# atlas-jj/ORB-SLAM-free-space-carving

Hardware: AMD Instinct MI355X
Metric: Mpix*KF/s fused (640x480xN_KF) (higher is better)
Workload: dtype f32

## Files before the change

### orb-slam-free-space-carving_amd/csrc/sdm_device.h

```cpp
#pragma once
#include <hip/hip_runtime.h>
#include <float.h>
#include <stddef.h>
#include <stdint.h>

#include "sdm_c.h"

namespace sdm {

struct KfMeta {
    float fx, fy, cx, cy;
    float Tcw[12];
    float I_stddev;
    int uploaded;
    int pad[2];
};

struct RefConst {
    int slot;
    float fx, fy, cx, cy;
    float mind, maxd;
    int act_count;
};

// ... 271 lines not shown
    return __builtin_fmaf(e, r, r);
}

#ifndef SDM_K1_OPT_ATAN_RCP
#define SDM_K1_OPT_ATAN_RCP 1
#endif
__device__ __forceinline__ float fast_atan2_deg_x1(float y)
{
    const float scale = (float)(180.0 / 3.14159265358979323846);
    const float p1 = 0.9997878412794807f * scale;
    const float p3 = -0.3258083974640975f * scale;
    const float p5 = 0.1555786518463281f * scale;
    const float p7 = -0.04432655554792128f * scale;
    float ay = fabsf(y);
    float a, c, c2;
    if (1.0f >= ay) {
        c = ay;
        c2 = c * c;
        a = (((p7 * c2 + p5) * c2 + p3) * c2 + p1) * c;
    } else {
#if SDM_K1_OPT_ATAN_RCP
        c = rcp_exact(ay + (float)DBL_EPSILON);
#else
        c = 1.0f / (ay + (float)DBL_EPSILON);
#endif
        c2 = c * c;
        a = 90.f - (((p7 * c2 + p5) * c2 + p3) * c2 + p1) * c;
    }
    if (y < 0) a = 360.f - a;
    return a;
}

#ifndef SDM_K1_OPT
#define SDM_K1_OPT 0x17fa27f
#endif

constexpr int PCV_FLOATS = 20;
constexpr int CV_RX = 9, CV_RZ = 12, CV_TX = 15, CV_TZ = 16, CV_ROT = 17, CV_ISTD = 18;
static_assert(offsetof(PairConst, Rx) == 4 * CV_RX && offsetof(PairConst, Rz) == 4 * CV_RZ && offsetof(PairConst, tx) == 4 * CV_TX &&
                  offsetof(PairConst, tz) == 4 * CV_TZ && offsetof(PairConst, rot) == 4 * CV_ROT &&
                  offsetof(PairConst, istd) == 4 * CV_ISTD && offsetof(PairConst, Ry) == 4 * PCV_FLOATS,
              "the CV_* indices follow PairConst");

__device__ __forceinline__ float match_cost1(float pe2, float ge2, const DevParams& prm)
{
    double s = (double)pe2 + (double)ge2 * prm.inv_theta;
    const unsigned lo = (unsigned)__double2loint(s), hi = (unsigned)__double2hiint(s);
    const bool risky = (((lo & 0x1FFFFFFFu) - 0x0FFFFF00u) <= 0x200u) | ((hi - 0x39C00000u) >= (0x46200000u - 0x39C00000u));
    if (__builtin_expect(risky, 0)) s = (double)pe2 + (double)ge2 / prm.theta_var;
    return (float)s;
}

constexpr float INV_THETA_DEFAULT_F = (float)(1.0 / 0.23);
constexpr unsigned COST_BAND = 16u;
__device__ __forceinline__ float match_cost_ref(float pe2, float ge2, const DevParams& prm)
{
    return (float)((double)pe2 + (double)ge2 / prm.theta_var);
}
__device__ __forceinline__ float match_cost_approx(float pe2, float ge2) { return __builtin_fmaf(ge2, INV_THETA_DEFAULT_F, pe2); }

__device__ __forceinline__ float lerp_w0(float yf)
{
#if SDM_K1_OPT & 0x10
    return 1.0f - __builtin_amdgcn_fractf(yf);
#else
    return (floorf(yf) + 1.0f) - yf;
#endif
// ... 179 lines not shown
    in = in && fx > 0.0f && fy > 0.0f && mind > 0.0f && maxd > 0.0f && tx != 0.0f && W >= 2 && H >= 2 && W <= 65536 && H <= 65536;
    if (!in) return 0;
    const Box xp0 = box_out((0.0f - cx) / fx, ((float)(W - 1) - cx) / fx);
    const Box xp1 = box_out((0.0f - cy) / fy, ((float)(H - 1) - cy) / fy);
    const Box rxxp = box_add(box_add(box_mul(box_pt(Rx[0]), xp0), box_mul(box_pt(Rx[1]), xp1)), box_pt(Rx[2]));
    const Box rzxp = box_add(box_add(box_mul(box_pt(Rz[0]), xp0), box_mul(box_pt(Rz[1]), xp1)), box_pt(Rz[2]));
    int bits = 0;
    {
        bool ok = fx * 0x1p-25f * fabsf(tx) * (1.0f - 0x1p-20f) >= QB_NUM_LO;
        const float ds[2] = {mind, maxd};
        for (int k = 0; k < 2; k++) {
            const Box xk = box_add(box_mul(rxxp, box_pt(ds[k])), box_pt(tx));
            const Box zk = box_add(box_mul(rzxp, box_pt(ds[k])), box_pt(tz));
            ok = ok && box_divisor_ok(zk) && box_mag_hi(box_mul(box_pt(fx), xk)) <= QB_NUM_HI;
        }
        if (ok) bits |= 8;
    }
    {
        const float w = (float)W;
        const Box ucx = box_add(Box{-QB_U_SPAN * w, (QB_U_SPAN + 1.0f) * w}, box_pt(-cx));
        const Box num = box_add(box_mul(rzxp, ucx), box_neg(box_mul(box_pt(fx), rxxp)));
        const Box den = box_add(box_mul(box_pt(-tz), ucx), box_mul(box_pt(fx), box_pt(tx)));
        const float nvar = 2 * istd * istd;
        const float lb = fminf(0x1p-50f * fx * fabsf(Rx[2]), rzxp.lo * 0x1p-25f * fabsf(cx)) * (1.0f - 0x1p-20f);
        bool ok = box_divisor_ok(den) && box_mag_hi(num) <= QB_NUM_HI && Rx[2] != 0.0f && cx != 0.0f && rzxp.lo >= 0x1p-10f &&
                  lb >= QB_NUM_LO && quot_input_ok(istd) && istd > 0.0f && nvar >= QB_NUM_LO && nvar <= QB_NUM_HI;
        const float root = (1002.0f + 1.4143f * istd) / (QB_U_SPAN * w) * (1.0f + 0x1p-10f);
        const unsigned eb = max((__float_as_uint(root * root) >> 23) + 1u, 97u);
        ok = ok && eb < (QB_DWIN_END >> 23);
        if (ok) bits |= 16 | (int)(eb << 8);
    }
    return bits;
}

struct ScanState {
    float old_err, best_pe, best_ge;
    int best_pixel;
};

struct ScanConst {
    const char* nbase;
    unsigned W16;
    float hlim_b;
    float ab, cb, pixel, grad1, th_line, ang_pi_rot, gate_lim;
    int hi;
};
template <bool STATS, bool CLEAN>
__device__ __forceinline__ void scan_candidate(const ScanConst& q, int uj, float yf, const float4& r, const DevParams& prm,
                                               ScanState& S, SearchStats* st)
{
    if (r.x < prm.lambdaG) return;
#if SDM_ABLATE == 4
    if (r.z > S.old_err) { S.best_pixel = uj; S.old_err = r.z; }
    return;
#endif
    const float d2 = r.y - q.th_line;
    const float d3 = r.y - q.ang_pi_rot;
    bool fail;
    if (CLEAN) {
#if SDM_K1_OPT & 0x04
        fail = gate2_fails_fast1(d2) | gate3_fails_fast1(d3);
#else
        fail = gate2_fails_fast(d2) | gate3_fails_fast(d3);
#endif
    } else {
        fail = gate2_fails_k(d2, prm.g2c) | gate3_fails_k(d3, prm.g3lo, prm.g3span);
// ... 530 lines not shown
    t_one = 1.0 / s2;
    const bool safe = (s2 > 1.0e-60) & (s2 < 1.0e60) & (ar > 1.0e-30f) & (ar < 1.0e30f);
    t_rho = safe ? div_by_with_rcp((double)rho, s2, t_one) : (double)rho / s2;
#endif
}
__device__ __forceinline__ void fusion_accum(float rho, float sg, float& pjsj, float& rsj)
{
    double t_rho, t_one;
    fusion_terms(rho, sg, t_rho, t_one);
    pjsj = (float)((double)pjsj + t_rho);
    rsj = (float)((double)rsj + t_one);
}
constexpr unsigned FD_SG_LO = 77u << 23, FD_SG_END = 177u << 23;
__device__ __forceinline__ bool fusion_accum_try(float rho, float sg, float& pjsj, float& rsj)
{
    if ((__float_as_uint(sg) - FD_SG_LO) >= (FD_SG_END - FD_SG_LO)) return false;
    const double sd = (double)sg;
    const double y = rcp_newton_f64(sd * sd, __builtin_amdgcn_rcpf(sg * sg));
    float np, nr;
    const bool okp = decided_sum((double)pjsj, (double)rho * y, np);
    const bool okr = decided_sum((double)rsj, y, nr);
    if (!(okp & okr)) return false;
    pjsj = np;
    rsj = nr;
    return true;
}
__device__ __forceinline__ void fusion_accum_decided(float rho, float sg, float& pjsj, float& rsj)
{
#if SDM_K1_OPT & 0x400000
    if (fusion_accum_try(rho, sg, pjsj, rsj)) return;
#endif
    fusion_accum(rho, sg, pjsj, rsj);
}

__device__ __forceinline__ float2 fusion_tail_ref(float pjsj, float rsj) { return make_float2(pjsj / rsj, sqrtf(1 / rsj)); }
__device__ __forceinline__ bool fusion_tail_window(float pjsj, float rsj)
{
    return ((__float_as_uint(pjsj) - QUOT_MAG_LO) <= (QUOT_MAG_HI - QUOT_MAG_LO)) &
           ((__float_as_uint(rsj) - QUOT_MAG_LO) <= (QUOT_MAG_HI - QUOT_MAG_LO));
}
__device__ __forceinline__ float2 fusion_tail_fast(float pjsj, float rsj)
{
    const float r = rcp_fast(rsj);
    const float rs = __builtin_amdgcn_rsqf(r);
    const float y0 = r * rs, hs = 0.5f * rs;
    return make_float2(quot_fast(pjsj, rsj, r), __builtin_fmaf(__builtin_fmaf(-y0, y0, r), hs, y0));
}
__device__ __forceinline__ float2 fusion_tail(float pjsj, float rsj)
{
#if SDM_K1_OPT & 0x800000
    if (fusion_tail_window(pjsj, rsj)) return fusion_tail_fast(pjsj, rsj);
#endif
    return fusion_tail_ref(pjsj, rsj);
}

__device__ __forceinline__ bool gt_1em6(float x) { return x > __uint_as_float(0x358637bdu); }
__device__ __forceinline__ bool lt_1em6(float x) { return x <= __uint_as_float(0x358637bdu); }

__device__ __forceinline__ float safe_rcp_sq(float s)
{
    float s2 = s * s;
    bool ok = (s2 >= 1.0e-30f) && (s2 <= 1.0e30f);
    return ok ? __builtin_amdgcn_rcpf(s2) : __builtin_nanf("");
}

__device__ __forceinline__ bool chi_test_fast(float a, float b, float sa, float sb, float ra, float rb)
// ... 10 lines not shown
{
    float d = ha.x - hb.x;
    float num = d * d;
    float approx = num * ha.y + num * hb.y;
    if (approx < 5.9896f) return true;
    if (approx > 5.9904f) return false;
    return chi_test(ha.x, hb.x, sa, *sb_ptr);
}

__device__ __forceinline__ bool fuse_column(const float2* hyp, int stride, int nh, int lambdaN,
                                            float& rho_o, float& sigma_o)
{
    unsigned long long bestmask = 0;
    int best = 0;
    for (int a = 0; a < nh; a++) {
        float2 ha = hyp[a * stride];
        const float ra = safe_rcp_sq(ha.y);
        unsigned long long m = 0;
        for (int b = 0; b < nh; b++) {
            float2 hb = hyp[b * stride];
            if (chi_test_fast(ha.x, hb.x, ha.y, hb.y, ra, safe_rcp_sq(hb.y))) m |= 1ull << b;
        }
        int cnt = __popcll(m);
        if (cnt > best) {
            best = cnt;
            bestmask = m;
        }
    }
    if (best < lambdaN) return false;
    float pjsj = 0.f, rsj = 0.f;
    for (int b = 0; b < nh; b++) {
        if (!((bestmask >> b) & 1ull)) continue;
        float2 hb = hyp[b * stride];
        fusion_accum_decided(hb.x, hb.y, pjsj, rsj);
    }
    const float2 res = fusion_tail(pjsj, rsj);
    rho_o = res.x;
    sigma_o = res.y;
    return true;
}

}
```

### orb-slam-free-space-carving_amd/csrc/sdm_engine.hip

```cpp
#include <hip/hip_runtime.h>

#include <algorithm>
#include <atomic>
#include <chrono>
#include <cmath>
#include <condition_variable>
#include <cstdio>
#include <cstdlib>
#include <cstring>
#include <limits>
#include <map>
#include <mutex>
#include <string>
#include <thread>
#include <new>
#include <vector>

#include "sdm_c.h"
#include "sdm_kernels.h"
#include "sdm_extract.h"
#include "sdm_support.h"
#include "sdm_priors.h"
#include "sdm_covis.h"
#include "sdm_voxel.h"
// ... 2546 lines not shown
        if (hipMalloc(&d_pc, sizeof(PairConst) * blocks * BLOCK) != hipSuccess) {
            (void)hipFree(d_patch);
            return fail(SDM_EHIP, "selftest scratch allocation failed");
        }
        hipLaunchKernelGGL(k_selftest_k4, dim3(blocks), dim3(BLOCK), 0, c->stream, 2048, d_patch, d_pc, c->d_stats + 5,
                           c->d_stats + 6, which == 9 ? 1 : 0);
        hipError_t e = hipGetLastError();
        if (e == hipSuccess) e = hipMemcpyAsync(out, c->d_stats + 5, sizeof(unsigned long long) * 2, hipMemcpyDeviceToHost, c->stream);
        if (e == hipSuccess) e = hipStreamSynchronize(c->stream);
        (void)hipFree(d_patch);
        (void)hipFree(d_pc);
        if (e != hipSuccess) return fail(SDM_EHIP, hipGetErrorString(e));
        HIP_TRY(hipMemsetAsync(c->d_stats, 0, sizeof(unsigned long long) * STATS_WORDS, c->stream));
        return SDM_OK;
    } else if (which == 6) {
        hipLaunchKernelGGL(k_selftest_rcp, dim3(4096), dim3(BLOCK), 0, c->stream, c->d_stats + 5, c->d_stats + 6);
    } else if (which == 8) {
        hipLaunchKernelGGL(k_selftest_scan_ids, dim3(4096), dim3(BLOCK), 0, c->stream, c->d_stats + 5, c->d_stats + 6);
    } else if (which == 10) {
        hipLaunchKernelGGL(k_selftest_atan_x1, dim3(4096), dim3(BLOCK), 0, c->stream, c->d_stats + 5, c->d_stats + 6);
    } else if (which == 3) {
        hipLaunchKernelGGL(k_selftest_gates, dim3(4096), dim3(BLOCK), 0, c->stream, c->dprm, c->d_stats + 5, c->d_stats + 6);
    } else if (which == 11) {
        hipLaunchKernelGGL(k_selftest_quot_boxes, dim3(4096), dim3(BLOCK), 0, c->stream, 4096, c->d_stats + 5, c->d_stats + 6);
    } else if (which == 13) {
        hipLaunchKernelGGL(k_selftest_ustar, dim3(ST_DEC_BLOCKS), dim3(BLOCK), 0, c->stream, c->dprm.inv_theta, ST13_ITERS,
                           c->d_stats + 5, c->d_stats + 6);
    } else if (which == 14) {
        hipLaunchKernelGGL(k_selftest_fusion_decided, dim3(ST_DEC_BLOCKS), dim3(BLOCK), 0, c->stream, ST14_ITERS, c->d_stats + 5,
                           c->d_stats + 6);
    } else if (which == 15) {
        hipLaunchKernelGGL(k_selftest_fusion_tail, dim3(ST_DEC_BLOCKS), dim3(BLOCK), 0, c->stream, ST15_ITERS, c->d_stats + 5,
                           c->d_stats + 6);
    } else if (which == 12) {
        const sdm_ctx::TableKey& key = c->sets[c->cur_set].key;
        if (!key.valid || !key.has_consts || !c->d_pairs) return fail(SDM_EINVAL, "no pair constants staged");
        const int np = key.n_ref * key.n;
        hipLaunchKernelGGL(k_selftest_pair_bits, dim3((np + BLOCK - 1) / BLOCK), dim3(BLOCK), 0, c->stream, c->d_pairs, np,
                           c->d_stats + 5, c->d_stats + 6);
    } else if (which == 16 || which == 17 || which == 18) {
        const unsigned long long* keys = nullptr;
        unsigned long long cap = 0;
        if (which == 18) {
            if (!c->vox_last_keys) return fail(SDM_ESTATE, "no per-call voxel table: sdm_extract_points_voxel* first");
            keys = c->vox_last_keys, cap = c->vox_last_cap;
        } else {
            if (!c->vmap.open) return fail(SDM_ESTATE, "no open voxel map");
            if (which == 16) keys = c->vmap.tb.keys, cap = c->vmap.cap;
            else if (c->vmap.obs.d_table) keys = c->vmap.obs.tb.keys, cap = c->vmap.obs.cap;
        }
        if (cap)
            launch_sliced(c, (long long)((cap + BLOCK - 1) / BLOCK), [&](long long b0, unsigned g) {
                hipLaunchKernelGGL(k_selftest_table_layout, dim3(g), dim3(BLOCK), 0, c->stream, keys, cap,
                                   (unsigned long long)b0 * BLOCK, c->d_stats + 5);
            });
    } else {
        return fail(SDM_EINVAL, "unknown selftest");
    }
    HIP_TRY(hipGetLastError());
    HIP_TRY(hipMemcpyAsync(out, c->d_stats + 5, sizeof(unsigned long long) * 2, hipMemcpyDeviceToHost, c->stream));
    HIP_TRY(hipStreamSynchronize(c->stream));
    HIP_TRY(hipMemsetAsync(c->d_stats, 0, sizeof(unsigned long long) * STATS_WORDS, c->stream));
    return SDM_OK;
}

int sdm_enable_timing(sdm_ctx* c, int on)
{
    if (!c) return fail(SDM_EINVAL, "null context");
    c->timing_on = on != 0;
    return SDM_OK;
}

// ... 75 lines not shown
```

### orb-slam-free-space-carving_amd/csrc/sdm_kernels.h

```cpp
#pragma once
#include "sdm_device.h"
#include "sdm_ingest.h"

namespace sdm {

#ifndef SDM_INTRA_COMPACT
#define SDM_INTRA_COMPACT 1
#endif

struct TileGeom {
    int W, H, tiles_x, tiles_y, ntiles;
};

__host__ __device__ inline TileGeom make_geom(int W, int H)
{
    TileGeom g;
    g.W = W;
    g.H = H;
    g.tiles_x = (W + TILE_W - 1) / TILE_W;
    g.tiles_y = (H + TILE_H - 1) / TILE_H;
    g.ntiles = g.tiles_x * g.tiles_y;
    return g;
}
__host__ inline int grid_blocks(const TileGeom& g, int n_ref) { return 8 * ((g.ntiles + 7) / 8) * n_ref; }
// ... 109 lines not shown
    if (idx >= n_ref * n) return;
    int r = idx / n, j = idx - r * n;
    KfMeta m1 = meta[ref_slots[r]];
    KfMeta m2 = meta[nbr_slots[idx]];
    PairConst pc;
    float R21[9], t21[3];
    pair_geometry(m1, m2, pc.F, R21, t21);
    for (int i = 0; i < 3; i++) {
        pc.Rx[i] = R21[i];
        pc.Ry[i] = R21[3 + i];
        pc.Rz[i] = R21[6 + i];
    }
    pc.tx = t21[0];
    pc.ty = t21[1];
    pc.tz = t21[2];
    pc.rot = rot ? rot[idx] : 0.0f;
    pc.istd = m2.I_stddev;
    pc.nbr_slot = nbr_slots[idx];
    pc.nfx = m2.fx;
    pc.nfy = m2.fy;
    pc.ncx = m2.cx;
    pc.ncy = m2.cy;
    pc.clean = ((theta_bad[ref_slots[r]] == 0 && theta_bad[nbr_slots[idx]] == 0 && pc.rot >= -360.0f && pc.rot <= 360.0f) ? 1 : 0) |
               (line_quot_safe(pc.F) ? 2 : 0);
    {
        float umin, umax;
        search_range(m1.fx, m1.cx, pc.Rx[2], pc.Rz[2], pc.tx, pc.tz, mind ? mind[r] : 0.f, maxd ? maxd[r] : 0.f, W, umin, umax);
        if (!(umax - umin < (float)MASK_HINT_L)) pc.clean |= 4;
    }
#if SDM_K1_OPT & 0x1c0000
    pc.clean |= quot_boxes(pc.Rx, pc.Rz, pc.tx, pc.tz, pc.istd, m1.fx, m1.fy, m1.cx, m1.cy, mind ? mind[r] : 0.f, maxd ? maxd[r] : 0.f,
                           W, H);
#endif
    {
        const float s = 1.0f + 0x1p-20f;
        const float X0 = fmaxf(fabsf(m1.cx), fabsf((float)(W - 1) - m1.cx)) / fabsf(m1.fx) * s;
        const float X1 = fmaxf(fabsf(m1.cy), fabsf((float)(H - 1) - m1.cy)) / fabsf(m1.fy) * s;
        k4_proj_bounds(pc, X0, X1);
    }
    pairs[idx] = pc;
    if (j == 0) {
        RefConst rc;
        rc.slot = ref_slots[r];
        rc.fx = m1.fx;
        rc.fy = m1.fy;
        rc.cx = m1.cx;
        rc.cy = m1.cy;
        rc.mind = mind ? mind[r] : 0.f;
        rc.maxd = maxd ? maxd[r] : 0.f;
        rc.act_count = act_counts[ref_slots[r]];
        refs[r] = rc;
    }
}

__global__ void k_ref_setup(const KfMeta* __restrict__ meta, const int* __restrict__ ref_slots,
                            const int* __restrict__ act_counts, int n_ref, RefConst* __restrict__ refs)
{
    int r = blockIdx.x * blockDim.x + threadIdx.x;
    if (r >= n_ref) return;
    KfMeta m = meta[ref_slots[r]];
    RefConst rc;
    rc.slot = ref_slots[r];
    rc.fx = m.fx;
    rc.fy = m.fy;
    rc.cx = m.cx;
    rc.cy = m.cy;
// ... 50 lines not shown
        const float sa = sgm[a * K1_PX + p];
        unsigned c = (sa * sa > 0.0f) ? 1u : 0u;
        for (int bb = a + 1; bb < n; bb++) {
            const float2 hb = hyp[bb * K1_PX + p];
            if (chi_test_lazy(ha, hb, sa, &sgm[bb * K1_PX + p])) {
                c++;
                atomicAdd(&cnt[(bb >> 2) * K1_PX + p], 1u << (8 * (bb & 3)));
            }
        }
        atomicAdd(&cnt[(a >> 2) * K1_PX + p], c << (8 * (a & 3)));
    }
}
__device__ __forceinline__ bool k1_fuse_counted(const float2* hyp, const float* sgm, const unsigned* cnt, unsigned long long vm,
                                                int n, int p, int lambdaN, float2& result)
{
    unsigned best = 0;
    int besta = 0;
    for (int a = 0; a < n; a++) {
        if (!((vm >> a) & 1ull)) continue;
        const unsigned c = (cnt[(a >> 2) * K1_PX + p] >> (8 * (a & 3))) & 0xffu;
        if (c > best) {
            best = c;
            besta = a;
        }
    }
    if ((int)best < lambdaN) return false;
    const float2 ha = hyp[besta * K1_PX + p];
    const float sa = sgm[besta * K1_PX + p];
    float pjsj = 0.f, rsj = 0.f;
    for (int bb = 0; bb < n; bb++) {
        if (!((vm >> bb) & 1ull)) continue;
        const float2 hb = hyp[bb * K1_PX + p];
        const bool in = (bb == besta) ? (sa * sa > 0.0f) : chi_test_lazy(ha, hb, sa, &sgm[bb * K1_PX + p]);
        if (in) fusion_accum_decided(hb.x, sgm[bb * K1_PX + p], pjsj, rsj);
    }
    result = fusion_tail(pjsj, rsj);
    return true;
}

#ifndef SDM_K1_EU_MIN
#define SDM_K1_EU_MIN 8
#endif
#ifndef SDM_K1_LB
#define SDM_K1_LB __launch_bounds__(K1_BLOCK) __attribute__((amdgpu_waves_per_eu(SDM_K1_EU_MIN, 8)))
#endif
template <bool STATS, bool MASK>
__global__ SDM_K1_LB void k_search_fuse(const float4* __restrict__ rec, long long plane,
                                                       const RefConst* __restrict__ refs,
                                                       const PairConst* __restrict__ pairs, int n_ref, int n,
                                                       int W, int H, int max_chunks, DevParams prm,
                                                       const unsigned* __restrict__ act, float2* __restrict__ pool,
                                                       unsigned long long* __restrict__ stats, OpenList open_list,
                                                       const unsigned* __restrict__ gmask, int mrow)
{
    extern __shared__ __align__(16) unsigned char smem_raw[];
    float2* hyp = reinterpret_cast<float2*>(smem_raw);
    float* sgm = reinterpret_cast<float*>(hyp + (size_t)n * K1_PX);
    unsigned* cnt = reinterpret_cast<unsigned*>(sgm + (size_t)n * K1_PX);
    const int cnt_words = max((n + 3) >> 2, K1_OUTLIER_ROWS);
    unsigned long long* pmask = reinterpret_cast<unsigned long long*>(cnt + (size_t)cnt_words * K1_PX);
    unsigned long long* set0 = pmask + K1_BLOCK;
    unsigned* cnt0 = reinterpret_cast<unsigned*>(set0 + K1_PX);
    unsigned* xbase = cnt0 + K1_PX;

    const int b = blockIdx.x;
    const int i8 = b >> 3;
    const int cl = i8 / n_ref;
    const int ref = i8 - cl * n_ref;
    const int chunk = cl * 8 + (b & 7);
    if (chunk >= max_chunks) return;
    const RefConst rc = refs[ref];
    if (chunk * K1_PX >= rc.act_count) return;
    const int tid = threadIdx.x, p = tid & (K1_PX - 1);
    const int w = __builtin_amdgcn_readfirstlane(tid >> 6);
    const int t = chunk * K1_PX + p;
    const bool on = t < rc.act_count;
    const float4* __restrict__ rrec = rec + (long long)rc.slot * plane;

    int x = 2, y = 2;
    float pixel = 0.f, grad1 = 0.f, th_pi = 0.f, xp0 = 0.f, xp1 = 0.f;
    if (on) {
        unsigned xy = act[(long long)rc.slot * plane + t];
        x = (int)(xy & 0xffffu);
        y = (int)(xy >> 16);
        float4 r = rrec[y * W + x];
        pixel = (float)(int)(__float_as_uint(r.w) & 0xffu);
        grad1 = r.x;
        th_pi = r.y;
        xp0 = ((float)x - rc.cx) / rc.fx;
        xp1 = ((float)y - rc.cy) / rc.fy;
    }
    SearchStats st = {0, 0, 0};
    MaskStats ms = {0, 0, 0};
    MaskView mv;
    mv.row_pitch = (unsigned)mrow * MASK_WORD_BYTES;
    const PairConst* __restrict__ pcs = pairs + (long long)ref * n;
    const float rcvb[4] = {rc.fx, rc.cx, rc.mind, rc.maxd};
    const float* __restrict__ rcv = rcvb;
    unsigned long long mymask = 0;
    for (int j = w; j < n; j += K1_WAVES) {
        const PairConst* __restrict__ pc = pcs + j;
        const float4* __restrict__ nrec = rec + (long long)pc->nbr_slot * plane;
        float2 h = make_float2(__builtin_inff(), 1.0f);
#if SDM_K1_OPT & 0x1000
        {
            float rho, sigma, bu, bv;
            const float* __restrict__ cv = reinterpret_cast<const float*>(pc);
            bool ok = epipolar_search<STATS, true>(nrec, W, H, cv, rcv, pc->clean, on, x, y, pixel, grad1, th_pi, xp0, xp1, prm,
                                                   rho, sigma, bu, bv, &st);
            if (ok && __float_as_uint(rho) < 0x7f800000u) {
                h = make_float2(rho, sigma);
                mymask |= 1ull << j;
            }
        }
#else
        if (on) {
            float rho, sigma, bu, bv;
            const float* __restrict__ cv = reinterpret_cast<const float*>(pc);
            mv.base = (MASK && gmask) ? reinterpret_cast<const char*>(gmask + (long long)pc->nbr_slot * H * MASK_PLANES * mrow) : nullptr;
            bool ok = epipolar_search<STATS, false, MASK>(nrec, W, H, cv, rcv, pc->clean, true, x, y, pixel, grad1, th_pi, xp0, xp1, prm, rho,
                                             sigma, bu, bv, &st, mv, &ms);
            if (ok && __float_as_uint(rho) < 0x7f800000u) {
                h = make_float2(rho, sigma);
                mymask |= 1ull << j;
            }
        }
#endif
        hyp[j * K1_PX + p] = make_float2(h.x, safe_rcp_sq(h.y));
        sgm[j * K1_PX + p] = h.y;
    }
    for (int q = w; q < cnt_words; q += K1_WAVES) cnt[q * K1_PX + p] = 0u;
    if (w == 0) {
        set0[p] = 0ull;
        cnt0[p] = 0u;
    }
    pmask[tid] = mymask;
    __syncthreads();

    unsigned long long vm = 0;
#pragma unroll
    for (int q = 0; q < K1_WAVES; q++) vm |= pmask[q * K1_PX + p];
#if SDM_ABLATE == 1
    const int nh = 0;
    if (vm == 0x123456789ull) pool[0] = make_float2(1.f, 1.f);
#else
    const int nh = __popcll(vm);
#endif
    const bool go = nh > prm.lambdaN;
    const int a0 = (int)__ffsll((long long)vm) - 1;
    bool self0 = false;
    if (go) {
        const float2 ha = hyp[a0 * K1_PX + p];
        const float sa = sgm[a0 * K1_PX + p];
        self0 = sa * sa > 0.0f;
        unsigned c = 0;
        for (int bb = w; bb < n; bb += K1_WAVES) {
            const float2 hb = hyp[bb * K1_PX + p];
            if (bb != a0 && chi_test_lazy(ha, hb, sa, &sgm[bb * K1_PX + p])) c++;
        }
        if (c) atomicAdd(&cnt0[p], c);
    }
    __syncthreads();
#if SDM_ABLATE == 9
    bool settled = false;
    const bool few = false;
    const unsigned long long S0 = 0ull;
    const int s0 = 0;
#else
    bool settled = go && self0 && (int)cnt0[p] + 1 == nh;
    const bool more = go && !settled && self0;
    unsigned long long S0 = settled ? vm : 0ull;
    if (__builtin_amdgcn_ballot_w64(more) != 0ull) {
        if (more) {
            const float2 ha = hyp[a0 * K1_PX + p];
            const float sa = sgm[a0 * K1_PX + p];
            unsigned long long m = 0;
            for (int bb = w; bb < n; bb += K1_WAVES) {
                const float2 hb = hyp[bb * K1_PX + p];
                if (bb != a0 && chi_test_lazy(ha, hb, sa, &sgm[bb * K1_PX + p])) m |= 1ull << bb;
            }
            if (m) atomicOr(&set0[p], m);
        }
        __syncthreads();
        if (more) S0 = set0[p] | (1ull << a0);
    }
    const int s0 = __popcll(S0);
    const unsigned long long O = vm & ~S0;
    const bool few = more && __popcll(O) <= K1_OUTLIER_ROWS;
    if (__builtin_amdgcn_ballot_w64(few) != 0ull) {
        unsigned* orow = cnt;
        unsigned long long rem = few ? O : 0ull;
        for (int i = 0; i < K1_OUTLIER_ROWS && __builtin_amdgcn_ballot_w64(rem != 0ull) != 0ull; i++) {
            if (rem != 0ull) {
                const int o = (int)__ffsll((long long)rem) - 1;
                rem &= rem - 1ull;
                const float2 ho = hyp[o * K1_PX + p];
                const float so = sgm[o * K1_PX + p];
                unsigned c = (w == 0 && so * so > 0.0f) ? 1u : 0u;
                for (int bb = w; bb < n; bb += K1_WAVES) {
                    const float2 hb = hyp[bb * K1_PX + p];
                    if (bb != o && chi_test_lazy(ho, hb, so, &sgm[bb * K1_PX + p])) c += ((S0 >> bb) & 1ull) ? 0x10001u : 1u;
                }
                if (c) atomicAdd(&orow[i * K1_PX + p], c);
            }
        }
        __syncthreads();
        if (few) {
            bool stands = true;
            const int nO = __popcll(O);
            for (int i = 0; i < K1_OUTLIER_ROWS; i++) {
                const unsigned v = orow[i * K1_PX + p];
                if (i < nO) stands = stands && (v >> 16) == 0u && (int)(v & 0xffffu) <= s0;
            }
            settled = stands;
        }
        __syncthreads();
        for (int q = w; q < K1_OUTLIER_ROWS; q += K1_WAVES) cnt[q * K1_PX + p] = 0u;
    }
#endif
    const bool open = go && !settled;
    const unsigned long long open_mask = __builtin_amdgcn_ballot_w64(open);
    bool deferred = false;
    if (open_mask != 0ull) {
        if (tid == 0) {
            const unsigned cntw = (unsigned)__popcll(open_mask);
            unsigned first = 0xFFFFFFFFu;
            if (cntw < open_list.inplace_min && atomicAdd(&open_list.count[0], cntw) >= open_list.quota) {
                const unsigned base = atomicAdd(&open_list.count[2], cntw);
                if (base <= open_list.capacity && cntw <= open_list.capacity - base)
                    first = base;
                else
                    atomicMin(&open_list.count[1], base);
            }
            xbase[0] = first;
        }
        __syncthreads();
        const unsigned base = xbase[0];
        deferred = base != 0xFFFFFFFFu;
        if (deferred) {
            if (open) {
                const unsigned e = base + (unsigned)__popcll(open_mask & ((1ull << p) - 1ull));
                float2* __restrict__ dst = open_list.hyp + ((size_t)(e >> 6) * n) * K1_PX + (e & 63u);
                for (int j = w; j < n; j += K1_WAVES) dst[(size_t)j * K1_PX] = make_float2(hyp[j * K1_PX + p].x, sgm[j * K1_PX + p]);
                if (w == 0) {
                    open_list.pix[e] = (long long)rc.slot * plane + y * W + x;
                    open_list.vm[e] = vm;
                }
            }
        } else {
            if (open) k1_count_all_pairs(hyp, sgm, cnt, vm, n, p, w);
            __syncthreads();
        }
    }

    unsigned long long n_fused = 0;
    if (w == 0 && on && !(open && deferred)) {
        float2 result = make_float2(0.f, 0.f);
        if (settled) {
            if (s0 >= prm.lambdaN) {
                float pjsj = 0.f, rsj = 0.f;
                for (int bb = 0; bb < n; bb++) {
                    if (!((S0 >> bb) & 1ull)) continue;
                    fusion_accum_decided(hyp[bb * K1_PX + p].x, sgm[bb * K1_PX + p], pjsj, rsj);
                }
                result = fusion_tail(pjsj, rsj);
                n_fused = 1;
            }
        } else if (go) {
            n_fused = k1_fuse_counted(hyp, sgm, cnt, vm, n, p, prm.lambdaN, result) ? 1 : 0;
        }
        pool[(long long)rc.slot * plane + y * W + x] = result;
    }
    if (STATS) {
        unsigned long long v[9] = {st.searches, st.candidates, st.gate_pass,
                                   (w == 0 && on) ? (unsigned long long)nh : 0ull, n_fused, ms.waves, ms.steps, ms.row_mismatch,
                                   (w == 0 && open) ? 1ull : 0ull};
#pragma unroll
        for (int k = 0; k < 9; k++) {
            unsigned long long s = v[k];
            for (int o = 32; o > 0; o >>= 1) s += __shfl_down(s, o);
            if ((tid & 63) == 0 && s) atomicAdd(&stats[k], s);
        }
    }
}

template <bool STATS>
__global__ __launch_bounds__(K1_BLOCK) void k_fuse_open(OpenList open_list, int n, DevParams prm, float2* __restrict__ pool,
                                                        long long pool_elems, unsigned long long* __restrict__ stats)
{
    extern __shared__ __align__(16) unsigned char smem_raw[];
    float2* hyp = reinterpret_cast<float2*>(smem_raw);
    float* sgm = reinterpret_cast<float*>(hyp + (size_t)n * K1_PX);
    unsigned* cnt = reinterpret_cast<unsigned*>(sgm + (size_t)n * K1_PX);
    const int cnt_words = (n + 3) >> 2;
    const unsigned total = min(min(open_list.count[2], open_list.count[1]), open_list.capacity);
    const int tid = threadIdx.x, p = tid & (K1_PX - 1);
// ... 654 lines not shown
    *slow = (g.lo < K4_MAG_LO) | (g.hi > K4_MAG_HI) | (amb != 0u) | (t_lo < K4_TAP_LO) |
            (t_hi > K4_TAP_HI) | (absbits(rzxp) >= 0x49800000u );
    return K4Sums{in.kf_count + nj, nsJr, nsJJ};
}
__device__ __forceinline__ K4Sums inter_neighbour_fast(const float2* __restrict__ nb, const PairConst* __restrict__ pc,
                                                       int W, float colsm1, float rowsm1, float xp0, float xp1,
                                                       float depthp, float dp, const K4Guard& g0, K4Sums in,
                                                       bool* slow)
{
    const K4Proj P = inter_project_any(pc, W, colsm1, rowsm1, xp0, xp1, depthp, dp, g0);
    const K4Rows R = inter_fetch(nb, W, P.off);
#if SDM_K4_NBRSKIP
    {
        const float lim = P.valid ? __uint_as_float(0x358637bdu) : __builtin_inff();
        const bool anyc = (R.ra.r0 > lim) | (R.rb.r0 > lim) | (R.ra.r1 > lim) | (R.rb.r1 > lim);
        if (__builtin_amdgcn_ballot_w64(anyc) == 0ull) {
            *slow = false;
            return in;
        }
    }
#endif
    return inter_taps(pc, P, R, depthp, dp, in, slow);
}

#ifndef SDM_K4_PIPE
#define SDM_K4_PIPE 0
#endif
__device__ __forceinline__ float inter_check_pixel(const float2* __restrict__ pool,
                                                   long long plane, const RefConst& rc,
                                                   const PairConst* __restrict__ pcs, int n, int W, int H, int x,
                                                   int y, float depthp, int lambdaN)
{
    const float colsm1 = (float)(W - 1), rowsm1 = (float)(H - 1);
    const float xp0 = ((float)x - rc.cx) / rc.fx, xp1 = ((float)y - rc.cy) / rc.fy;
    const float dp = rcp_exact(depthp);
    K4Guard g0 = {absbits(depthp), absbits(depthp)};
    K4Sums acc = {0, 0.f, 0.f};
#if SDM_K4_PIPE
    K4Proj P = inter_project_any(pcs, W, colsm1, rowsm1, xp0, xp1, depthp, dp, g0);
    K4Rows R = inter_fetch(pool + (long long)pcs->nbr_slot * plane, W, P.off);
    for (int j = 0; j < n; j++) {
        const PairConst* __restrict__ pc = pcs + j;
        const float2* __restrict__ nb = pool + (long long)pc->nbr_slot * plane;
        const PairConst* __restrict__ pcn = pcs + min(j + 1, n - 1);
        const K4Proj Pn = inter_project_any(pcn, W, colsm1, rowsm1, xp0, xp1, depthp, dp, g0);
        const K4Rows Rn = inter_fetch(pool + (long long)pcn->nbr_slot * plane, W, Pn.off);
        bool slow;
        const K4Sums fast = inter_taps(pc, P, R, depthp, dp, acc, &slow);
        if (__builtin_expect(slow, 0))
            acc = inter_neighbour_exact(nb, pc, W, colsm1, rowsm1, xp0, xp1, depthp, dp, acc);
        else
            acc = fast;
        P = Pn;
        R = Rn;
    }
#else
#if SDM_K4_CPRE
    PairConst nxt = pcs[0];
    for (int j = 0; j < n; j++) {
        const PairConst cur = nxt;
        if (j + 1 < n) nxt = pcs[j + 1];
        const float2* __restrict__ nb = pool + (long long)cur.nbr_slot * plane;
        bool slow;
        const K4Sums fast = inter_neighbour_fast(nb, &cur, W, colsm1, rowsm1, xp0, xp1, depthp, dp, g0, acc, &slow);
        if (__builtin_expect(slow, 0))
            acc = inter_neighbour_exact(nb, pcs + j, W, colsm1, rowsm1, xp0, xp1, depthp, dp, acc);
        else
// ... 799 lines not shown
                if (!st_same_bits(got.x, want.x) || !st_same_bits(got.y, want.y)) cnt++;
            } else {
                und++;
            }
        }
        if ((pick & 3u) != 0) continue;
        switch ((pick >> 2) & 7u) {
        case 0: a = __uint_as_float(__float_as_uint(a) | 0x7FFFFFu); break;
        case 1: b = __uint_as_float(__float_as_uint(b) | 0x7FFFFFu); break;
        case 2: a = __uint_as_float(__float_as_uint(a) | 0x7FFFFFu); b = __uint_as_float(__float_as_uint(b) | 0x7FFFFFu); break;
        case 3: a = sp[(pick >> 8) % 12u]; break;
        case 4: b = sp[(pick >> 8) % 12u]; break;
        case 5: a = sp[(pick >> 8) % 12u]; b = sp[(pick >> 12) % 12u]; break;
        default: {
            const float k = (float)(1u + ((pick >> 8) & 255u));
            a = __uint_as_float(__float_as_uint(k * b) + ((pick >> 16) & 3u) - 1u);
            break;
        }
        }
        const float2 want = fusion_tail_ref(a, b);
        const float2 got = fusion_tail_window(a, b) ? fusion_tail_fast(a, b) : fusion_tail(a, b);
        if (!st_same_bits(got.x, want.x) || !st_same_bits(got.y, want.y)) cnt++;
    }
    for (int o = 32; o > 0; o >>= 1) {
        cnt += __shfl_down(cnt, o);
        und += __shfl_down(und, o);
    }
    if ((threadIdx.x & 63) == 0) {
        if (cnt) atomicAdd(bad, cnt);
        if (und) atomicAdd(undecided, und);
    }
}

__global__ __launch_bounds__(BLOCK) void k_selftest_gates(DevParams prm, unsigned long long* __restrict__ bad,
                                                          unsigned long long* __restrict__ tested)
{
    const unsigned gid = blockIdx.x * BLOCK + threadIdx.x, nthreads = gridDim.x * BLOCK;
    unsigned long long cnt = 0, n = 0;
    auto check = [&](float d) {
        if (!(d < 360.0f)) return;
        if (prm.default_gates) {
            if (gate2_fails_fast(d) != gate2_fails_ref(d, 80.0f)) cnt++;
            if (gate3_fails_fast(d) != gate3_fails_ref(d, 45.0f)) cnt++;
            if (gate2_fails_fast1(d) != gate2_fails_ref(d, 80.0f)) cnt++;
            if (gate3_fails_fast1(d) != gate3_fails_ref(d, 45.0f)) cnt++;
        }
        if (gate2_fails_k(d, prm.g2c) != gate2_fails_ref(d, prm.lambdaL)) cnt++;
        if (gate3_fails_k(d, prm.g3lo, prm.g3span) != gate3_fails_ref(d, prm.lambdaTheta)) cnt++;
        n++;
    };
    for (unsigned u = gid; u <= 0x43C80000u; u += nthreads) {
        check(__uint_as_float(u));
        check(__uint_as_float(u | 0x80000000u));
    }
    const float bnd[12] = {0.f, 45.f, 80.f, 90.f, 100.f, 180.f, 260.f, 270.f, 280.f, 315.f, 360.f, 135.f};
    if (gid < 12 * 4096) {
        unsigned base = __float_as_uint(bnd[gid / 4096]);
        int k = (int)(gid % 4096) - 2048;
        float v = __uint_as_float(base + k);
        check(v);
        check(-v);
    }
    unsigned s = 0xC2B2AE35u * (gid + 1);
    for (int i = 0; i < 64; i++) {
        float t2 = ((xs32(s) >> 8) * (1.0f / 16777216.0f)) * 360.0f;
        float rf = ((xs32(s) >> 8) * (1.0f / 16777216.0f)) * 360.0f;
// ... 15 lines not shown
```

Before: 14440.

## Add seeded fusion accumulate, fast pixel-ray quotient, and skip LDS clears when settled

Enables three new optimization bits by default. The fusion accumulation reuses the already-computed reciprocal-square of sigma stored in the hypothesis table as a Newton seed instead of recomputing it. The per-pixel normalized coordinates use a fast reciprocal quotient when a per-pair guard bit shows that the camera intrinsics fall in a safe range. The LDS count and set clears and the extra barrier are deferred and skipped entirely when no pixel in the block is still unsettled. Self-test kernels are added for the new paths. This adds branches and guard logic and carries a risk of exactness bugs outside the tested ranges.

Measured after the change: 14580, median of 6. No clear change (+1.0%).

```diff
diff --git a/orb-slam-free-space-carving_amd/csrc/sdm_device.h b/orb-slam-free-space-carving_amd/csrc/sdm_device.h
--- a/orb-slam-free-space-carving_amd/csrc/sdm_device.h
+++ b/orb-slam-free-space-carving_amd/csrc/sdm_device.h
@@ -327,7 +327,7 @@
 }
 
 #ifndef SDM_K1_OPT
-#define SDM_K1_OPT 0x17fa27f
+#define SDM_K1_OPT 0xf7fa27f
 #endif
 
 constexpr int PCV_FLOATS = 20;
@@ -573,6 +573,20 @@
     }
     return bits;
 }
+
+#ifndef SDM_K4_XPQUOT
+#define SDM_K4_XPQUOT 0
+#endif
+constexpr int CLEAN_XPQUOT = 32;
+__device__ inline bool xp_quot_ok(float fx, float fy, float cx, float cy, int W, int H)
+{
+    const unsigned mx = absbits(fx), my = absbits(fy), nx = absbits(cx), ny = absbits(cy);
+    const unsigned d_lo = (127u - 30u) << 23, d_hi = (127u + 20u) << 23, n_lo = (127u - 36u) << 23;
+    return mx >= d_lo && mx <= d_hi && my >= d_lo && my <= d_hi && (nx == 0u || (nx >= n_lo && nx <= d_hi)) &&
+           (ny == 0u || (ny >= n_lo && ny <= d_hi)) && W >= 1 && H >= 1 && W <= 65536 && H <= 65536;
+}
+__device__ __forceinline__ float xp_ref(int x, float c, float f) { return ((float)x - c) / f; }
+__device__ __forceinline__ float xp_fast(int x, float c, float f) { return quot_fast((float)x - c, f, rcp_fast(f)); }
 
 struct ScanState {
     float old_err, best_pe, best_ge;
@@ -1169,6 +1183,28 @@
 #endif
     fusion_accum(rho, sg, pjsj, rsj);
 }
+__device__ __forceinline__ bool fusion_accum_try_seeded(float rho, float sg, float rs, float& pjsj, float& rsj)
+{
+    if (rs != rs) return false;
+    const double sd = (double)sg;
+    const double y = rcp_newton_f64(sd * sd, rs);
+    float np, nr;
+    const bool okp = decided_sum((double)pjsj, (double)rho * y, np);
+    const bool okr = decided_sum((double)rsj, y, nr);
+    if (!(okp & okr)) return false;
+    pjsj = np;
+    rsj = nr;
+    return true;
+}
+__device__ __forceinline__ void fusion_accum_seeded(float rho, float sg, float rs, float& pjsj, float& rsj)
+{
+#if (SDM_K1_OPT & 0x4400000) == 0x4400000
+    if (fusion_accum_try_seeded(rho, sg, rs, pjsj, rsj)) return;
+    fusion_accum(rho, sg, pjsj, rsj);
+#else
+    fusion_accum_decided(rho, sg, pjsj, rsj);
+#endif
+}
 
 __device__ __forceinline__ float2 fusion_tail_ref(float pjsj, float rsj) { return make_float2(pjsj / rsj, sqrtf(1 / rsj)); }
 __device__ __forceinline__ bool fusion_tail_window(float pjsj, float rsj)
@@ -1245,7 +1281,11 @@
     for (int b = 0; b < nh; b++) {
         if (!((bestmask >> b) & 1ull)) continue;
         float2 hb = hyp[b * stride];
+#if (SDM_K1_OPT & 0x4400000) == 0x4400000
+        fusion_accum_seeded(hb.x, hb.y, safe_rcp_sq(hb.y), pjsj, rsj);
+#else
         fusion_accum_decided(hb.x, hb.y, pjsj, rsj);
+#endif
     }
     const float2 res = fusion_tail(pjsj, rsj);
     rho_o = res.x;
diff --git a/orb-slam-free-space-carving_amd/csrc/sdm_engine.hip b/orb-slam-free-space-carving_amd/csrc/sdm_engine.hip
--- a/orb-slam-free-space-carving_amd/csrc/sdm_engine.hip
+++ b/orb-slam-free-space-carving_amd/csrc/sdm_engine.hip
@@ -2602,12 +2602,21 @@
     } else if (which == 15) {
         hipLaunchKernelGGL(k_selftest_fusion_tail, dim3(ST_DEC_BLOCKS), dim3(BLOCK), 0, c->stream, ST15_ITERS, c->d_stats + 5,
                            c->d_stats + 6);
-    } else if (which == 12) {
+    } else if (which == 19) {
+        hipLaunchKernelGGL(k_selftest_xp, dim3(4096), dim3(BLOCK), 0, c->stream, ST19_ITERS, c->d_stats + 5, c->d_stats + 6);
+    } else if (which == 20) {
+        hipLaunchKernelGGL(k_selftest_fusion_seeded, dim3(ST_DEC_BLOCKS), dim3(BLOCK), 0, c->stream, ST14_ITERS, c->d_stats + 5,
+                           c->d_stats + 6);
+    } else if (which == 12 || which == 21) {
         const sdm_ctx::TableKey& key = c->sets[c->cur_set].key;
         if (!key.valid || !key.has_consts || !c->d_pairs) return fail(SDM_EINVAL, "no pair constants staged");
         const int np = key.n_ref * key.n;
-        hipLaunchKernelGGL(k_selftest_pair_bits, dim3((np + BLOCK - 1) / BLOCK), dim3(BLOCK), 0, c->stream, c->d_pairs, np,
-                           c->d_stats + 5, c->d_stats + 6);
+        if (which == 12)
+            hipLaunchKernelGGL(k_selftest_pair_bits, dim3((np + BLOCK - 1) / BLOCK), dim3(BLOCK), 0, c->stream, c->d_pairs, np,
+                               c->d_stats + 5, c->d_stats + 6);
+        else
+            hipLaunchKernelGGL(k_selftest_pair_xp, dim3((np + BLOCK - 1) / BLOCK), dim3(BLOCK), 0, c->stream, c->d_pairs, np,
+                               c->d_stats + 5, c->d_stats + 6);
     } else if (which == 16 || which == 17 || which == 18) {
         const unsigned long long* keys = nullptr;
         unsigned long long cap = 0;
diff --git a/orb-slam-free-space-carving_amd/csrc/sdm_kernels.h b/orb-slam-free-space-carving_amd/csrc/sdm_kernels.h
--- a/orb-slam-free-space-carving_amd/csrc/sdm_kernels.h
+++ b/orb-slam-free-space-carving_amd/csrc/sdm_kernels.h
@@ -165,6 +165,9 @@
     pc.clean |= quot_boxes(pc.Rx, pc.Rz, pc.tx, pc.tz, pc.istd, m1.fx, m1.fy, m1.cx, m1.cy, mind ? mind[r] : 0.f, maxd ? maxd[r] : 0.f,
                            W, H);
 #endif
+#if (SDM_K1_OPT & 0x8000000) || SDM_K4_XPQUOT
+    if (xp_quot_ok(m1.fx, m1.fy, m1.cx, m1.cy, W, H)) pc.clean |= CLEAN_XPQUOT;
+#endif
     {
         const float s = 1.0f + 0x1p-20f;
         const float X0 = fmaxf(fabsf(m1.cx), fabsf((float)(W - 1) - m1.cx)) / fabsf(m1.fx) * s;
@@ -281,7 +284,7 @@
         if (!((vm >> bb) & 1ull)) continue;
         const float2 hb = hyp[bb * K1_PX + p];
         const bool in = (bb == besta) ? (sa * sa > 0.0f) : chi_test_lazy(ha, hb, sa, &sgm[bb * K1_PX + p]);
-        if (in) fusion_accum_decided(hb.x, sgm[bb * K1_PX + p], pjsj, rsj);
+        if (in) fusion_accum_seeded(hb.x, sgm[bb * K1_PX + p], hb.y, pjsj, rsj);
     }
     result = fusion_tail(pjsj, rsj);
     return true;
@@ -328,6 +331,9 @@
 
     int x = 2, y = 2;
     float pixel = 0.f, grad1 = 0.f, th_pi = 0.f, xp0 = 0.f, xp1 = 0.f;
+#if SDM_K1_OPT & 0x8000000
+    const bool xpq = n > 0 && (pairs[(long long)ref * n].clean & CLEAN_XPQUOT) != 0;
+#endif
     if (on) {
         unsigned xy = act[(long long)rc.slot * plane + t];
         x = (int)(xy & 0xffffu);
@@ -336,8 +342,16 @@
         pixel = (float)(int)(__float_as_uint(r.w) & 0xffu);
         grad1 = r.x;
         th_pi = r.y;
-        xp0 = ((float)x - rc.cx) / rc.fx;
-        xp1 = ((float)y - rc.cy) / rc.fy;
+#if SDM_K1_OPT & 0x8000000
+        if (xpq) {
+            xp0 = xp_fast(x, rc.cx, rc.fx);
+            xp1 = xp_fast(y, rc.cy, rc.fy);
+        } else
+#endif
+        {
+            xp0 = ((float)x - rc.cx) / rc.fx;
+            xp1 = ((float)y - rc.cy) / rc.fy;
+        }
     }
     SearchStats st = {0, 0, 0};
     MaskStats ms = {0, 0, 0};
@@ -378,11 +392,15 @@
         hyp[j * K1_PX + p] = make_float2(h.x, safe_rcp_sq(h.y));
         sgm[j * K1_PX + p] = h.y;
     }
+#if SDM_K1_OPT & 0x2000000
+    if (w == 0) cnt0[p] = 0u;
+#else
     for (int q = w; q < cnt_words; q += K1_WAVES) cnt[q * K1_PX + p] = 0u;
     if (w == 0) {
         set0[p] = 0ull;
         cnt0[p] = 0u;
     }
+#endif
     pmask[tid] = mymask;
     __syncthreads();
 
@@ -412,95 +430,108 @@
     __syncthreads();
 #if SDM_ABLATE == 9
     bool settled = false;
-    const bool few = false;
-    const unsigned long long S0 = 0ull;
-    const int s0 = 0;
+    unsigned long long S0 = 0ull;
 #else
     bool settled = go && self0 && (int)cnt0[p] + 1 == nh;
-    const bool more = go && !settled && self0;
     unsigned long long S0 = settled ? vm : 0ull;
-    if (__builtin_amdgcn_ballot_w64(more) != 0ull) {
-        if (more) {
-            const float2 ha = hyp[a0 * K1_PX + p];
-            const float sa = sgm[a0 * K1_PX + p];
-            unsigned long long m = 0;
-            for (int bb = w; bb < n; bb += K1_WAVES) {
-                const float2 hb = hyp[bb * K1_PX + p];
-                if (bb != a0 && chi_test_lazy(ha, hb, sa, &sgm[bb * K1_PX + p])) m |= 1ull << bb;
-            }
-            if (m) atomicOr(&set0[p], m);
-        }
+#endif
+    bool open = false, deferred = false;
+#if SDM_K1_OPT & 0x2000000
+    const bool busy = __builtin_amdgcn_ballot_w64(go && !settled) != 0ull;
+    if (busy) {
+        for (int q = w; q < cnt_words; q += K1_WAVES) cnt[q * K1_PX + p] = 0u;
+        if (w == 0) set0[p] = 0ull;
         __syncthreads();
-        if (more) S0 = set0[p] | (1ull << a0);
-    }
-    const int s0 = __popcll(S0);
-    const unsigned long long O = vm & ~S0;
-    const bool few = more && __popcll(O) <= K1_OUTLIER_ROWS;
-    if (__builtin_amdgcn_ballot_w64(few) != 0ull) {
-        unsigned* orow = cnt;
-        unsigned long long rem = few ? O : 0ull;
-        for (int i = 0; i < K1_OUTLIER_ROWS && __builtin_amdgcn_ballot_w64(rem != 0ull) != 0ull; i++) {
-            if (rem != 0ull) {
-                const int o = (int)__ffsll((long long)rem) - 1;
-                rem &= rem - 1ull;
-                const float2 ho = hyp[o * K1_PX + p];
-                const float so = sgm[o * K1_PX + p];
-                unsigned c = (w == 0 && so * so > 0.0f) ? 1u : 0u;
+    }
+    if (busy)
+#endif
+    {
+#if SDM_ABLATE != 9
+        const bool more = go && !settled && self0;
+        if (__builtin_amdgcn_ballot_w64(more) != 0ull) {
+            if (more) {
+                const float2 ha = hyp[a0 * K1_PX + p];
+                const float sa = sgm[a0 * K1_PX + p];
+                unsigned long long m = 0;
                 for (int bb = w; bb < n; bb += K1_WAVES) {
                     const float2 hb = hyp[bb * K1_PX + p];
-                    if (bb != o && chi_test_lazy(ho, hb, so, &sgm[bb * K1_PX + p])) c += ((S0 >> bb) & 1ull) ? 0x10001u : 1u;
+                    if (bb != a0 && chi_test_lazy(ha, hb, sa, &sgm[bb * K1_PX + p])) m |= 1ull << bb;
                 }
-                if (c) atomicAdd(&orow[i * K1_PX + p], c);
+                if (m) atomicOr(&set0[p], m);
             }
-        }
-        __syncthreads();
-        if (few) {
-            bool stands = true;
-            const int nO = __popcll(O);
-            for (int i = 0; i < K1_OUTLIER_ROWS; i++) {
-                const unsigned v = orow[i * K1_PX + p];
-                if (i < nO) stands = stands && (v >> 16) == 0u && (int)(v & 0xffffu) <= s0;
-            }
-            settled = stands;
-        }
-        __syncthreads();
-        for (int q = w; q < K1_OUTLIER_ROWS; q += K1_WAVES) cnt[q * K1_PX + p] = 0u;
-    }
-#endif
-    const bool open = go && !settled;
-    const unsigned long long open_mask = __builtin_amdgcn_ballot_w64(open);
-    bool deferred = false;
-    if (open_mask != 0ull) {
-        if (tid == 0) {
-            const unsigned cntw = (unsigned)__popcll(open_mask);
-            unsigned first = 0xFFFFFFFFu;
-            if (cntw < open_list.inplace_min && atomicAdd(&open_list.count[0], cntw) >= open_list.quota) {
-                const unsigned base = atomicAdd(&open_list.count[2], cntw);
-                if (base <= open_list.capacity && cntw <= open_list.capacity - base)
-                    first = base;
-                else
-                    atomicMin(&open_list.count[1], base);
-            }
-            xbase[0] = first;
-        }
-        __syncthreads();
-        const unsigned base = xbase[0];
-        deferred = base != 0xFFFFFFFFu;
-        if (deferred) {
-            if (open) {
-                const unsigned e = base + (unsigned)__popcll(open_mask & ((1ull << p) - 1ull));
-                float2* __restrict__ dst = open_list.hyp + ((size_t)(e >> 6) * n) * K1_PX + (e & 63u);
-                for (int j = w; j < n; j += K1_WAVES) dst[(size_t)j * K1_PX] = make_float2(hyp[j * K1_PX + p].x, sgm[j * K1_PX + p]);
-                if (w == 0) {
-                    open_list.pix[e] = (long long)rc.slot * plane + y * W + x;
-                    open_list.vm[e] = vm;
+            __syncthreads();
+            if (more) S0 = set0[p] | (1ull << a0);
+        }
+        const int s0 = __popcll(S0);
+        const unsigned long long O = vm & ~S0;
+        const bool few = more && __popcll(O) <= K1_OUTLIER_ROWS;
+        if (__builtin_amdgcn_ballot_w64(few) != 0ull) {
+            unsigned* orow = cnt;
+            unsigned long long rem = few ? O : 0ull;
+            for (int i = 0; i < K1_OUTLIER_ROWS && __builtin_amdgcn_ballot_w64(rem != 0ull) != 0ull; i++) {
+                if (rem != 0ull) {
+                    const int o = (int)__ffsll((long long)rem) - 1;
+                    rem &= rem - 1ull;
+                    const float2 ho = hyp[o * K1_PX + p];
+                    const float so = sgm[o * K1_PX + p];
+                    unsigned c = (w == 0 && so * so > 0.0f) ? 1u : 0u;
+                    for (int bb = w; bb < n; bb += K1_WAVES) {
+                        const float2 hb = hyp[bb * K1_PX + p];
+                        if (bb != o && chi_test_lazy(ho, hb, so, &sgm[bb * K1_PX + p])) c += ((S0 >> bb) & 1ull) ? 0x10001u : 1u;
+                    }
+                    if (c) atomicAdd(&orow[i * K1_PX + p], c);
                 }
             }
-        } else {
-            if (open) k1_count_all_pairs(hyp, sgm, cnt, vm, n, p, w);
             __syncthreads();
-        }
-    }
+            if (few) {
+                bool stands = true;
+                const int nO = __popcll(O);
+                for (int i = 0; i < K1_OUTLIER_ROWS; i++) {
+                    const unsigned v = orow[i * K1_PX + p];
+                    if (i < nO) stands = stands && (v >> 16) == 0u && (int)(v & 0xffffu) <= s0;
+                }
+                settled = stands;
+            }
+            __syncthreads();
+            for (int q = w; q < K1_OUTLIER_ROWS; q += K1_WAVES) cnt[q * K1_PX + p] = 0u;
+        }
+#endif
+        open = go && !settled;
+        const unsigned long long open_mask = __builtin_amdgcn_ballot_w64(open);
+        if (open_mask != 0ull) {
+            if (tid == 0) {
+                const unsigned cntw = (unsigned)__popcll(open_mask);
+                unsigned first = 0xFFFFFFFFu;
+                if (cntw < open_list.inplace_min && atomicAdd(&open_list.count[0], cntw) >= open_list.quota) {
+                    const unsigned base = atomicAdd(&open_list.count[2], cntw);
+                    if (base <= open_list.capacity && cntw <= open_list.capacity - base)
+                        first = base;
+                    else
+                        atomicMin(&open_list.count[1], base);
+                }
+                xbase[0] = first;
+            }
+            __syncthreads();
+            const unsigned base = xbase[0];
+            deferred = base != 0xFFFFFFFFu;
+            if (deferred) {
+                if (open) {
+                    const unsigned e = base + (unsigned)__popcll(open_mask & ((1ull << p) - 1ull));
+                    float2* __restrict__ dst = open_list.hyp + ((size_t)(e >> 6) * n) * K1_PX + (e & 63u);
+                    for (int j = w; j < n; j += K1_WAVES)
+                        dst[(size_t)j * K1_PX] = make_float2(hyp[j * K1_PX + p].x, sgm[j * K1_PX + p]);
+                    if (w == 0) {
+                        open_list.pix[e] = (long long)rc.slot * plane + y * W + x;
+                        open_list.vm[e] = vm;
+                    }
+                }
+            } else {
+                if (open) k1_count_all_pairs(hyp, sgm, cnt, vm, n, p, w);
+                __syncthreads();
+            }
+        }
+    }
+    const int s0 = __popcll(S0);
 
     unsigned long long n_fused = 0;
     if (w == 0 && on && !(open && deferred)) {
@@ -510,7 +541,8 @@
                 float pjsj = 0.f, rsj = 0.f;
                 for (int bb = 0; bb < n; bb++) {
                     if (!((S0 >> bb) & 1ull)) continue;
-                    fusion_accum_decided(hyp[bb * K1_PX + p].x, sgm[bb * K1_PX + p], pjsj, rsj);
+                    const float2 hb = hyp[bb * K1_PX + p];
+                    fusion_accum_seeded(hb.x, sgm[bb * K1_PX + p], hb.y, pjsj, rsj);
                 }
                 result = fusion_tail(pjsj, rsj);
                 n_fused = 1;
@@ -1231,7 +1263,18 @@
                                                    int y, float depthp, int lambdaN)
 {
     const float colsm1 = (float)(W - 1), rowsm1 = (float)(H - 1);
+#if SDM_K4_XPQUOT
+    float xp0, xp1;
+    if (n > 0 && (pcs->clean & CLEAN_XPQUOT)) {
+        xp0 = xp_fast(x, rc.cx, rc.fx);
+        xp1 = xp_fast(y, rc.cy, rc.fy);
+    } else {
+        xp0 = xp_ref(x, rc.cx, rc.fx);
+        xp1 = xp_ref(y, rc.cy, rc.fy);
+    }
+#else
     const float xp0 = ((float)x - rc.cx) / rc.fx, xp1 = ((float)y - rc.cy) / rc.fy;
+#endif
     const float dp = rcp_exact(depthp);
     K4Guard g0 = {absbits(depthp), absbits(depthp)};
     K4Sums acc = {0, 0.f, 0.f};
@@ -2097,6 +2140,114 @@
     }
 }
 
+constexpr int ST19_ITERS = 1024;
+__global__ __launch_bounds__(BLOCK) void k_selftest_xp(int iters, unsigned long long* __restrict__ bad,
+                                                       unsigned long long* __restrict__ tested)
+{
+    unsigned s = 0x27D4EB2Fu * (blockIdx.x * BLOCK + threadIdx.x + 1);
+    unsigned long long cnt = 0, n = 0;
+    const float out_f[8] = {0.f, 1e-41f, 0x1p-31f, 0x1.000002p20f, __builtin_inff(), __builtin_nanf(""), -0x1p-31f, -0x1p21f};
+    const float out_c[5] = {0x1p-37f, 0x1.000002p20f, __builtin_inff(), __builtin_nanf(""), -1e-41f};
+    for (int i = 0; i < iters; i++) {
+        const unsigned bf = xs32(s), bc = xs32(s), bx = xs32(s), pick = xs32(s);
+        float f = st_mag(bf, 97u, 50u, 0x80000000u);
+        if ((pick & 0xff00u) == 0u) f = (pick & 1u) ? 0x1p20f : -0x1p20f;
+        float c;
+        if (i & 1)
+            c = (float)(bc % (65536u * 16u)) * 0.0625f;
+        else if ((bc >> 29) == 0u)
+            c = (bc & 1u) ? 0.f : -0.f;
+        else
+            c = st_mag(bc, 91u, 56u, 0x80000000u);
+        int x = (int)(bx & 0xffffu);
+        if ((i & 3) == 3) x = min(max((int)c + (int)(bx % 5u) - 2, 0), 65535);
+        if (!xp_quot_ok(f, f, c, c, 65536, 65536) || !st_same_bits(xp_fast(x, c, f), xp_ref(x, c, f))) cnt++;
+        n++;
+        if ((pick & 15u) == 0u) {
+            const float fo = out_f[(pick >> 4) & 7u], co = out_c[(pick >> 7) % 5u];
+            if (xp_quot_ok(fo, f, c, c, 640, 480) || xp_quot_ok(f, fo, c, c, 640, 480) || xp_quot_ok(f, f, co, c, 640, 480) ||
+                xp_quot_ok(f, f, c, co, 640, 480) || xp_quot_ok(f, f, c, c, 65537, 480) || xp_quot_ok(f, f, c, c, 640, 65537))
+                cnt++;
+        }
+    }
+    for (int o = 32; o > 0; o >>= 1) {
+        cnt += __shfl_down(cnt, o);
+        n += __shfl_down(n, o);
+    }
+    if ((threadIdx.x & 63) == 0) {
+        if (cnt) atomicAdd(bad, cnt);
+        atomicAdd(tested, n);
+    }
+}
+
+__global__ __launch_bounds__(BLOCK) void k_selftest_pair_xp(const PairConst* __restrict__ pairs, int n_pairs,
+                                                            unsigned long long* __restrict__ with_bit,
+                                                            unsigned long long* __restrict__ tested)
+{
+    const int i = blockIdx.x * BLOCK + threadIdx.x;
+    if (i >= n_pairs) return;
+    if (pairs[i].clean & CLEAN_XPQUOT) atomicAdd(with_bit, 1ull);
+    atomicAdd(tested, 1ull);
+}
+
+__global__ __launch_bounds__(BLOCK) void k_selftest_fusion_seeded(int iters, unsigned long long* __restrict__ bad,
+                                                                  unsigned long long* __restrict__ undecided)
+{
+    unsigned s = 0x165667B1u * (blockIdx.x * BLOCK + threadIdx.x + 1);
+    unsigned long long cnt = 0, und = 0;
+    const float sg_sp[12] = {0x1p-50f, __uint_as_float(FD_SG_END - 1u), 0x1p-60f, 0x1p60f, 0.f, 1e-41f, __builtin_inff(),
+                             __builtin_nanf(""), -0.01f, 3e-39f, -0.f, -0x1p-60f};
+    const float rho_sp[6] = {0.f, -0.f, __builtin_inff(), __builtin_nanf(""), 1e-41f, -0.5f};
+    for (int i = 0; i < iters; i++) {
+        const int len = 1 + i % 20;
+        const float base = st_mag(xs32(s), 123u, 6u, 0u);
+        float pjsj = 0.f, rsj = 0.f;
+        for (int t = 0; t < len; t++) {
+            const unsigned br = xs32(s), bs = xs32(s);
+            const float rho = base * (1.0f + 0.01f * ((float)(br >> 8) * (2.0f / 16777216.0f) - 1.0f));
+            const float sg = st_mag(bs, 112u, 11u, 0u);
+            float wp = pjsj, wr = rsj, gp = pjsj, gr = rsj;
+            fusion_accum_plain(rho, sg, wp, wr);
+            if (fusion_accum_try_seeded(rho, sg, safe_rcp_sq(sg), gp, gr)) {
+                if (!st_same_bits(gp, wp) || !st_same_bits(gr, wr)) cnt++;
+            } else {
+                und++;
+            }
+            pjsj = wp;
+            rsj = wr;
+        }
+        const unsigned pick = xs32(s);
+        float sg = sg_sp[pick % 12u];
+        if ((pick >> 12) & 1u) {
+            const unsigned end = ((pick >> 13) & 1u) ? __float_as_uint(1e-15f) : __float_as_uint(1e15f);
+            sg = __uint_as_float(end + ((pick >> 14) % 9u) - 4u);
+            if ((pick >> 20) & 1u) sg = -sg;
+        }
+        const float rho = ((pick >> 8) & 1u) ? rho_sp[(pick >> 9) % 6u] : base;
+        const float rs = safe_rcp_sq(sg);
+        float wp = pjsj, wr = rsj, gp = pjsj, gr = rsj;
+        fusion_accum_plain(rho, sg, wp, wr);
+        if (fusion_accum_try_seeded(rho, sg, rs, gp, gr) && (!st_same_bits(gp, wp) || !st_same_bits(gr, wr))) cnt++;
+        gp = pjsj;
+        gr = rsj;
+        fusion_accum_seeded(rho, sg, rs, gp, gr);
+        if (!st_same_bits(gp, wp) || !st_same_bits(gr, wr)) cnt++;
+        if (rs == rs && !(fabsf(sg) > 0x1p-50f && fabsf(sg) < 0x1p50f)) cnt++;
+        float ap = pjsj, ar = rsj, bp = pjsj, br2 = rsj;
+        const bool da = fusion_accum_try_seeded(rho, fabsf(sg), safe_rcp_sq(fabsf(sg)), ap, ar);
+        const bool db = fusion_accum_try_seeded(rho, -fabsf(sg), safe_rcp_sq(-fabsf(sg)), bp, br2);
+        if (da != db || (da && (!st_same_bits(ap, bp) || !st_same_bits(ar, br2)))) cnt++;
+    }
+    for (int o = 32; o > 0; o >>= 1) {
+        cnt += __shfl_down(cnt, o);
+        und += __shfl_down(und, o);
+    }
+    if ((threadIdx.x & 63) == 0) {
+        if (cnt) atomicAdd(bad, cnt);
+        if (und) atomicAdd(undecided, und);
+    }
+}
+
 __global__ __launch_bounds__(BLOCK) void k_selftest_gates(DevParams prm, unsigned long long* __restrict__ bad,
                                                           unsigned long long* __restrict__ tested)
 {
```
